# frankyangdev/net.jgp.labs.sparkdq4ml

Hardware: AMD Instinct MI355X
Metric: rows/sec LinearRegression.fit, 1e8x32 synthetic, at 1/2/4/8 MI355X (higher is better)
Workload: dtype bf16; 1 GPU; model=LinearRegression(normal equations) d=32, global_batch=100000000, seq_len=32, parallelism=dp1, rows_per_gpu=100000000, device=cuda:0, storage=bf16, fit_mode=async

## Files before the change

net/jgp/labs/sparkdq4ml_amd/ops/csrc/hip/gram.h:

```cpp
#pragma once
#ifndef __HIPCC_RTC__
#include <hip/hip_runtime.h>

#include <cstdint>
#endif

namespace dq4ml {

enum GramMode : int { GRAM_F64 = 0, GRAM_F32 = 1, GRAM_BF16 = 2, GRAM_FP8 = 3, GRAM_F32S = 4 };

struct GramArgs {
  const void* X;
  int64_t ld;
  int d;
  int64_t n;
  int xdt;
  const void* y;
  int ydt;
  const void* w;
  int wdt;
  const uint8_t* sel;
  double* partials;
  int P;
  int64_t spw;
  int64_t nsuper;
  int tiled;
  const void* colp[8];
  int coldt[8];
  int cols;
  const int64_t* srcs;
  int interleave;
  const int64_t* rawtab;
  const float* xshift;
};

#ifndef __HIPCC_RTC__
int64_t tiled_elems(int d, int64_t n);

int gram_interleave();
void tile_bf16(const void* X, int xdt, int64_t ld, int d, int64_t n, void* out, hipStream_t st,
               const float* shift = nullptr);

int64_t gram_partial_stride(int mode, int d);
int gram_default_blocks(int64_t n);
int gram_plan_blocks(int mode, int d, int64_t n, int xdt, int xmode);
void gram_tall(int mode, GramArgs a, int xmode, int blocks, double* out, hipStream_t st, bool reduce = true);
void gram_reduce(int mode, const double* partials, int blocks, int d, double* out, hipStream_t st);
void stats_unshift(double* flat, const float* shift, int d, hipStream_t st);

void gram_window_fold(const double* part, int64_t rows, int gw, double* flat, hipStream_t st);

bool gram_stream_ok(int mode, const GramArgs& a);
int gram_stream_blocks(int mode, int d, int64_t n, int xdt);
void gram_stream(int mode, GramArgs a, int xmode, int blocks, double* out, hipStream_t st, bool reduce = true);

struct PackSrcG {
// ... 12 lines not shown
```

net/jgp/labs/sparkdq4ml_amd/ops/csrc/hip/gram.hip:

```cpp
#include <hip/hip_runtime.h>

#include <cstdlib>

#include "common.h"
#include "gram.h"

namespace dq4ml {

namespace {

constexpr int kBlock = 256;
constexpr int kWavesPerBlock = kBlock / kWave;
template <int NT, int XMODE, bool HALF = false>
struct BF16Geom {
  static constexpr int kBlock = (NT == 1 && XMODE == 0 && !HALF) ? 1024 : 512;
  static constexpr int kWaves = kBlock / kWave;
  static constexpr int kMinBlocks = HALF ? 2 : 1;
};
static int bf16_block(int, int) { return 512; }

__device__ __forceinline__ double load_as_f64(const void* p, int dt, int64_t i) {
  switch (dt) {
    case DT_F64: return reinterpret_cast<const double*>(p)[i];
    case DT_F32: return (double)reinterpret_cast<const float*>(p)[i];
// ... 14 lines not shown
  RowVals v{false, 0.0, 0.0, 0.0};
  if (r < a.n) {
    bool live = a.sel ? (a.sel[r] != 0) : true;
    if (live) {
      double w = a.w ? load_as_f64(a.w, a.wdt, r) : 1.0;
      double y = load_as_f64(a.y, a.ydt, r);
      v.live = true;
      v.w = w;
      v.y = y;
      v.wy = w * y;
    }
  }
  return v;
}

struct RowAcc {
  double cnt = 0, ws = 0, wws = 0, bs = 0, bbs = 0;
  __device__ __forceinline__ void add(const RowVals& v) {
    if (v.live) {
      cnt += 1.0;
      ws += v.w;
      wws += v.w * v.w;
      bs += v.wy;
      bbs += v.wy * v.y;
    }
  }
};

template <typename T>
__device__ __forceinline__ void load_rows32_bf16(const T* p, int64_t rows_left, bf16x8 (&fr)[4]);
// ... 80 lines not shown
  const int e = o - head, pr = e / (T * T), w = e - pr * T * T, r = w / T, cc = w - (w / T) * T;
  int I = 0, rem = pr;
  while (rem >= NT - I) {
    rem -= NT - I;
    ++I;
  }
  const int J = I + rem;
  const int64_t i = (int64_t)I * T + r, j = (int64_t)J * T + cc;
  if (i <= j && j < d) out[head + i + j * (j + 1) / 2] = t;
}

__device__ __forceinline__ void slab_put(double* p, double v) {
  __hip_atomic_store(p, v, __ATOMIC_RELAXED, __HIP_MEMORY_SCOPE_AGENT);
}

template <typename TX, int NT, int XMODE, bool TILED, bool HALF = false>
__global__ __launch_bounds__((BF16Geom<NT, XMODE, HALF>::kBlock), (BF16Geom<NT, XMODE, HALF>::kMinBlocks)) void
gram_tall_bf16_kernel(GramArgs a) {
  typedef BF16Geom<NT, XMODE, HALF> Geo;
  constexpr int NPAIR = NT * (NT + 1) / 2;
  extern __shared__ __attribute__((aligned(16))) unsigned char smem[];
  const int lane = threadIdx.x & 63;
  const int wave = threadIdx.x >> 6;
  const int f = lane & 31, h = lane >> 5;
  __bf16* wl = reinterpret_cast<__bf16*>(smem) + wave * (4 * 64);
  float* wrow = reinterpret_cast<float*>(smem + Geo::kWaves * 4 * 64 * 2) + wave * 64;

  f32x16 acc[NPAIR];
  f32x16 accw[NT];
#pragma unroll
  for (int p = 0; p < NPAIR; ++p) acc[p] = f32x16{};
#pragma unroll
  for (int t = 0; t < NT; ++t) accw[t] = f32x16{};
  RowAcc ra;

  const TX* X = reinterpret_cast<const TX*>(a.X);
  const TX* fp[NT];
  bool fvalid[NT];
#pragma unroll
  for (int t = 0; t < NT; ++t) {
    const int feat = t * 32 + f;
    fvalid[t] = feat < a.d;
    fp[t] = X + (int64_t)(fvalid[t] ? feat : 0) * a.ld + 32 * h;
  }

  const int64_t gw = (int64_t)blockIdx.x * Geo::kWaves + wave;
  const int64_t total_waves = (int64_t)gridDim.x * Geo::kWaves;
  int64_t s0 = gw * a.spw;
  int64_t s1 = s0 + a.spw;
  if (s1 > a.nsuper) s1 = a.nsuper;
  const bool do_tail = (gw == total_waves - 1) && (a.n > a.nsuper * 64);

  auto compute = [&](int64_t r0, bf16x8 (&fr)[NT][4]) {
    RowVals rv = row_vals(a, r0 + lane);
    ra.add(rv);
    {
      const float w_hi = (float)(__bf16)(float)rv.w;
      const __bf16 wy_hi = (__bf16)(float)rv.wy;
      wl[0 * 64 + lane] = (__bf16)(float)rv.w;
      wl[1 * 64 + lane] = (__bf16)(float)(rv.w - (double)w_hi);
      wl[2 * 64 + lane] = wy_hi;
      wl[3 * 64 + lane] = (__bf16)(float)(rv.wy - (double)(float)wy_hi);
      if (XMODE == 2) wrow[lane] = (float)rv.w;
    }
    const uint64_t live_bits = __ballot(rv.live);
    __builtin_amdgcn_wave_barrier();
    bf16x8 wf[4];
#pragma unroll
    for (int i = 0; i < 4; ++i) wf[i] = bf16x8{};
// ... 15 lines not shown
      for (int t = 0; t < NT; ++t) weight_frags(frw[t], wrow + 32 * h);
    }
    int p = 0;
#pragma unroll
    for (int I = 0; I < NT; ++I)
#pragma unroll
      for (int J = I; J < NT; ++J, ++p)
#pragma unroll
        for (int i = 0; i < 4; ++i) acc[p] = __builtin_amdgcn_mfma_f32_32x32x16_bf16(fr[I][i], frw[J][i], acc[p], 0, 0, 0);
#pragma unroll
    for (int t = 0; t < NT; ++t)
#pragma unroll
      for (int i = 0; i < 4; ++i) accw[t] = __builtin_amdgcn_mfma_f32_32x32x16_bf16(fr[t][i], wf[i], accw[t], 0, 0, 0);
    __builtin_amdgcn_wave_barrier();
  };
  auto load = [&](int64_t r0, int64_t rows_left, bf16x8 (&fr)[NT][4]) {
    if constexpr (TILED) {
      const u32x4* q = reinterpret_cast<const u32x4*>(a.X) + ((r0 >> 6) * NT) * 4 * 64 + lane;
#pragma unroll
      for (int t = 0; t < NT; ++t)
#pragma unroll
        for (int i = 0; i < 4; ++i) fr[t][i] = __builtin_bit_cast(bf16x8, __builtin_nontemporal_load(q + (t * 4 + i) * 64));
      return;
    }
#pragma unroll
    for (int t = 0; t < NT; ++t) {
      if (fvalid[t]) {
        load_rows32_bf16<TX>(fp[t] + r0, rows_left, fr[t]);
      } else {
#pragma unroll
        for (int i = 0; i < 4; ++i) fr[t][i] = bf16x8{};
      }
    }
  };

  if (a.interleave) {
    if (gw < a.nsuper) {
      bf16x8 cur[NT][4], nxt[NT][4];
      load(gw * 64, 64, cur);
      for (int64_t s = gw; s < a.nsuper; s += total_waves) {
        if (s + total_waves < a.nsuper) load((s + total_waves) * 64, 64, nxt);
        compute(s * 64, cur);
#pragma unroll
        for (int t = 0; t < NT; ++t)
#pragma unroll
          for (int i = 0; i < 4; ++i) cur[t][i] = nxt[t][i];
      }
    }
  } else if (s0 < s1) {
    bf16x8 cur[NT][4], nxt[NT][4];
    load(s0 * 64, 64, cur);
    for (int64_t s = s0; s < s1; ++s) {
      if (s + 1 < s1) load((s + 1) * 64, 64, nxt);
      compute(s * 64, cur);
#pragma unroll
      for (int t = 0; t < NT; ++t)
#pragma unroll
        for (int i = 0; i < 4; ++i) cur[t][i] = nxt[t][i];
    }
  }
  if (do_tail) {
    bf16x8 tl[NT][4];
    const int64_t r0 = a.nsuper * 64;
    load(r0, a.n - (r0 + 32 * h), tl);
    compute(r0, tl);
  }

  constexpr int W = Geo::kWaves;
  constexpr int NV = (NPAIR + NT) * 16;
  const int d = a.d;
  double sc[5] = {ra.cnt, ra.ws, ra.wws, ra.bs, ra.bbs};
#pragma unroll
  for (int k = 0; k < 5; ++k) sc[k] = wave_sum_f64(sc[k]);
  __syncthreads();
  float* tr = reinterpret_cast<float*>(smem);
  double* scl = reinterpret_cast<double*>(smem + (size_t)(W / 2) * NV * 64 * sizeof(float));
// ... 711 lines not shown
        for (int j = 0; j < 8; ++j) e[j] = (r + j < n) ? X[(int64_t)f * ld + r + j] : (uint16_t)0;
        v = __builtin_bit_cast(u32x4, e);
      }
      if (shift) {
        const float sh = shift[f];
        bf16x8 b = __builtin_bit_cast(bf16x8, v);
#pragma unroll
        for (int j = 0; j < 8; ++j) b[j] = (r + j < n) ? (__bf16)((float)b[j] - sh) : (__bf16)0.0f;
        v = __builtin_bit_cast(u32x4, b);
      }
    }
    reinterpret_cast<u32x4*>(out)[c] = v;
  }
}

__global__ __launch_bounds__(256) void unshift_aa_kernel(double* __restrict__ flat, const float* __restrict__ shift,
                                                        int d) {
  const double W = flat[1];
  const double* as = flat + 5;
  double* aa = flat + 5 + 2 * (int64_t)d;
  const int64_t tot = (int64_t)d * (d + 1) / 2;
  for (int64_t e = (int64_t)blockIdx.x * blockDim.x + threadIdx.x; e < tot; e += (int64_t)gridDim.x * blockDim.x) {
    int64_t j = (int64_t)((sqrt(8.0 * (double)e + 1.0) - 1.0) * 0.5);
    while (j * (j + 1) / 2 > e) --j;
    while ((j + 1) * (j + 2) / 2 <= e) ++j;
    const int64_t i = e - j * (j + 1) / 2;
    const double si = (double)shift[i], sj = (double)shift[j];
    aa[e] += si * as[j] + sj * as[i] + si * sj * W;
  }
}
// ... 31 lines not shown
  const int64_t nchunks = nsup * NT * 256;
  int64_t g = (nchunks + 255) / 256;
  if (g > 8192) g = 8192;
  if (g < 1) g = 1;
  uint16_t* o = reinterpret_cast<uint16_t*>(out);
  switch (xdt) {
    case DT_BF16: hipLaunchKernelGGL(tile_bf16_kernel<uint16_t>, dim3(g), dim3(256), 0, st, (const uint16_t*)X, ld, d, n, NT, nsup, o, shift); break;
    case DT_F32: hipLaunchKernelGGL(tile_bf16_kernel<float>, dim3(g), dim3(256), 0, st, (const float*)X, ld, d, n, NT, nsup, o, shift); break;
    case DT_F64: hipLaunchKernelGGL(tile_bf16_kernel<double>, dim3(g), dim3(256), 0, st, (const double*)X, ld, d, n, NT, nsup, o, shift); break;
    case DT_I32: hipLaunchKernelGGL(tile_bf16_kernel<int32_t>, dim3(g), dim3(256), 0, st, (const int32_t*)X, ld, d, n, NT, nsup, o, shift); break;
    default: throw std::invalid_argument("tile_bf16: unsupported dtype");
  }
  DQ_HIP_CHECK(hipGetLastError());
}

int64_t gram_partial_stride(int mode, int d) {
  if (mode == GRAM_F64) {
    const int NT = (d + 15) / 16;
    return 5 + 2 * (int64_t)d + (int64_t)NT * (NT + 1) / 2 * 256;
  }
  const int NT = (d + 31) / 32;
  return 5 + 2 * (int64_t)d + (int64_t)NT * (NT + 1) / 2 * 1024;
}

int gram_default_blocks(int64_t n) {
  const int64_t nsuper = (n + 63) / 64;
  int64_t blocks = (nsuper + 8 * kWavesPerBlock - 1) / (8 * kWavesPerBlock);
  if (blocks > 1024) blocks = 1024;
  if (blocks < 1) blocks = 1;
  return (int)blocks;
// ... 12 lines not shown
static size_t bf16_lds(int d, int xmode) {
  const int W = bf16_block(d, xmode) / kWave;
  const int NT = (d + 31) / 32;
  const size_t stripes = (size_t)W * (4 * 64 * 2 + 64 * 4);
  const size_t tree = (size_t)(W / 2) * ((NT * (NT + 1) / 2 + NT) * 16) * 64 * sizeof(float) + (size_t)W * 5 * 8;
  return tree > stripes ? tree : stripes;
}

static size_t f64_lds(int d) {
  size_t lds = kWavesPerBlock * (128 + 16 * kStageLd) * sizeof(double);
  const size_t red = (size_t)gram_partial_stride(GRAM_F64, d) * sizeof(double);
  return red > lds ? red : lds;
}

template <typename F>
static void with_kernel(int mode, int xdt, int d, int xmode, bool tiled, F&& f) {
  if (mode == GRAM_BF16) {
    const int NT = (d + 31) / 32;
#define DQ_BF16_CASE(TX, NTV, TL)                                                 \
    if (xmode == 0 && NTV == 1) return f(gram_tall_bf16_kernel<TX, 1, 0, TL, true>); \
    if (xmode == 0) return f(gram_tall_bf16_kernel<TX, NTV, 0, TL>);              \
    if (xmode == 1) return f(gram_tall_bf16_kernel<TX, NTV, 1, TL>);              \
    return f(gram_tall_bf16_kernel<TX, NTV, 2, TL>);
    if (xdt == DT_BF16 && tiled) { if (NT == 1) { DQ_BF16_CASE(uint16_t, 1, true) } else { DQ_BF16_CASE(uint16_t, 2, true) } }
    if (tiled) throw std::invalid_argument("gram_tall: tiled storage must be bf16");
    if (xdt == DT_BF16) { if (NT == 1) { DQ_BF16_CASE(uint16_t, 1, false) } else { DQ_BF16_CASE(uint16_t, 2, false) } }
    if (xdt == DT_F32) { if (NT == 1) { DQ_BF16_CASE(float, 1, false) } else { DQ_BF16_CASE(float, 2, false) } }
    if (xdt == DT_F64) { if (NT == 1) { DQ_BF16_CASE(double, 1, false) } else { DQ_BF16_CASE(double, 2, false) } }
#undef DQ_BF16_CASE
    throw std::invalid_argument("gram_tall(bf16): unsupported feature dtype");
  }
  if (mode == GRAM_F64) {
    const int NT = (d + 15) / 16;
#define DQ_F64_CASE(TX)                                        \
    switch (NT) {                                              \
      case 1: return f(gram_tall_f64_kernel<TX, 1>);           \
      case 2: return f(gram_tall_f64_kernel<TX, 2>);           \
      case 3: return f(gram_tall_f64_kernel<TX, 3>);           \
      default: return f(gram_tall_f64_kernel<TX, 4>);          \
    }
    if (xdt == DT_F64) { DQ_F64_CASE(double) }
    if (xdt == DT_F32) { DQ_F64_CASE(float) }
#undef DQ_F64_CASE
// ... 64 lines not shown
int gram_plan_blocks(int mode, int d, int64_t n, int xdt, int xmode) {
  if (mode == GRAM_F32 || mode == GRAM_F32S || (use_stream() && ((mode == GRAM_F64 && !use_skinny(mode, d, xdt, 0) &&
                                              (xdt == DT_F64 || xdt == DT_F32)) ||
                                             (mode == GRAM_BF16 && xdt == DT_F32))))
    return gram_stream_blocks(mode, d, n, xdt);
  if (use_skinny(mode, d, xdt, 0)) {
    int full = 1;
    with_skinny(xdt, d, [&](auto kern) { full = occupancy_blocks(kern, 0, kBlock); });
    int64_t want = (n + (int64_t)kBlock * 4 * 8 - 1) / ((int64_t)kBlock * 4 * 8);
    if (want < 1) want = 1;
    return (int)(want < full ? want : full);
  }
  const size_t lds = mode == GRAM_BF16 ? bf16_lds(d, xmode) : f64_lds(d);
  int full = 1;
  const int block = mode == GRAM_BF16 ? bf16_block(d, xmode) : kBlock;
  with_kernel(mode, xdt, d, xmode, false, [&](auto kern) { full = occupancy_blocks(kern, lds, block); });
  const int64_t nsuper = (n + 63) / 64;
  const int wpb = block / kWave;
  int64_t want = (nsuper + 4 * wpb - 1) / (4 * wpb);
  if (want < 1) want = 1;
  return (int)(want < full ? want : full);
}

void gram_window_fold(const double* part, int64_t rows, int gw, double* flat, hipStream_t st) {
  if (gw < 1 || rows < 0) throw std::invalid_argument("gram_window_fold: bad shape");
  hipLaunchKernelGGL(window_fold_kernel, dim3(gw), dim3(256), 0, st, part, rows, gw, flat);
  DQ_HIP_CHECK(hipGetLastError());
}

void gram_reduce(int mode, const double* partials, int blocks, int d, double* out, hipStream_t st) {
  const int T = mode == GRAM_F64 ? 16 : 32;
// ... 7 lines not shown
  return 1;
}

void gram_tall(int mode, GramArgs a, int xmode, int blocks, double* out, hipStream_t st, bool reduce) {
  if (a.d < 1 || a.d > 64) throw std::invalid_argument("gram_tall: d must be in [1, 64]");
  if (blocks < 1) throw std::invalid_argument("gram_tall: blocks must be >= 1");
  a.nsuper = a.n / 64;
  const int block = mode == GRAM_BF16 ? bf16_block(a.d, xmode) : kBlock;
  const int64_t total_waves = (int64_t)blocks * (block / kWave);
  a.spw = (a.nsuper + total_waves - 1) / total_waves;
  if (a.spw < 1) a.spw = 1;
  a.interleave = gram_interleave();
  a.P = (int)gram_partial_stride(mode, a.d);
  const size_t lds = mode == GRAM_BF16 ? bf16_lds(a.d, xmode) : f64_lds(a.d);
  if (a.tiled && mode != GRAM_BF16) throw std::invalid_argument("gram_tall: tiled storage needs bf16 mode");
  if (a.xshift) {
    if (!((mode == GRAM_F32 || mode == GRAM_BF16 || mode == GRAM_F32S) && a.xdt == DT_F32 && !a.tiled && a.cols == 0 &&
          gram_stream_ok(mode, a)))
      throw std::invalid_argument("gram_tall: a feature shift needs 16-byte aligned f32 features (stream kernel)");
    gram_stream(mode, a, 1, blocks, out, st, reduce);
    return;
  }
  if (a.cols > 0) {
    if (mode != GRAM_F64 || a.cols != a.d || a.d > kSkinnyMaxD || a.tiled)
      throw std::invalid_argument("gram_tall: columnar sources need f64 mode and d <= 8");
    with_skinny_cols(a, [&](auto kern) { hipLaunchKernelGGL(kern, dim3(blocks), dim3(kBlock), 0, st, a); });
  } else if (use_skinny(mode, a.d, a.xdt, a.tiled)) {
    with_skinny(a.xdt, a.d, [&](auto kern) { hipLaunchKernelGGL(kern, dim3(blocks), dim3(kBlock), 0, st, a); });
  } else if ((mode == GRAM_F32 || mode == GRAM_F32S ||
              (use_stream() && (mode == GRAM_F64 || (mode == GRAM_BF16 && a.xdt == DT_F32)))) &&
             gram_stream_ok(mode, a)) {
    gram_stream(mode, a, xmode, blocks, out, st, reduce);
    return;
  } else if (mode == GRAM_F32 || mode == GRAM_F32S) {
    throw std::invalid_argument("gram_tall(f32): needs 16-byte aligned f32 features and f32/f64 labels");
  } else {
    with_kernel(mode, a.xdt, a.d, xmode, a.tiled != 0,
                [&](auto kern) { hipLaunchKernelGGL(kern, dim3(blocks), dim3(block), lds, st, a); });
  }
  DQ_HIP_CHECK(hipGetLastError());
  if (reduce) gram_reduce(mode, a.partials, blocks, a.d, out, st);
}

static size_t cols_lds(int NT) {
  const size_t bufs = 2 * ((size_t)NT * 4 * 64 * 16 + 4 * 64 * 2);
  const size_t tree = (size_t)2 * ((NT * (NT + 1) / 2 + NT) * 16) * 64 * sizeof(float) + 4 * 5 * sizeof(double);
  return bufs > tree ? bufs : tree;
}

template <typename F>
static void with_cols_kernel(int NT, int sdt, int ydt, F&& f) {
#define DQ_COLS(NTV, YT)                                                 \
// ... 44 lines not shown
```

net/jgp/labs/sparkdq4ml_amd/ops/csrc/hip/module.cpp:

```cpp
#include <map>
#include <utility>
#include <vector>

#include <pybind11/pybind11.h>
#include <pybind11/stl.h>

#include "common.h"
#include "csv_scan.h"
#include "dqvm.h"
#include "gram.h"
#include "gram_folds.h"
#include "quantile.h"
#include "gram_wide.h"
#include "gram_syrk.h"
#include "wls_small.h"
#include "wls_large.h"
#include "rowops.h"
#include "lsq.h"

namespace py = pybind11;
using namespace dq4ml;

template <typename T>
static T* P(uintptr_t p) {
// ... 71 lines not shown
          a.tiled = tiled;
          a.xshift = P<const float>(xshift);
          a.X = P<const void>(X);
          a.ld = ld;
          a.d = d;
          a.n = n;
          a.xdt = xdt;
          a.y = P<const void>(y);
          a.ydt = ydt;
          a.w = P<const void>(w);
          a.wdt = wdt;
          a.sel = P<const uint8_t>(sel);
          a.partials = P<double>(partials);
          gram_tall(mode, a, xmode, blocks, P<double>(out), as_stream(stream), reduce);
        });
  m.def("gram_stream_cols",
        [](int mode, uintptr_t srcs, int d, int64_t n, int xdt, uintptr_t y, int ydt, uintptr_t w, int wdt,
           uintptr_t sel, uintptr_t partials, int blocks, uintptr_t out, uintptr_t stream, uintptr_t xshift) {
          GramArgs a{};
          a.srcs = P<const int64_t>(srcs);
          a.xshift = P<const float>(xshift);
          a.d = d;
          a.n = n;
          a.xdt = xdt;
          a.y = P<const void>(y);
          a.ydt = ydt;
          a.w = P<const void>(w);
          a.wdt = wdt;
          a.sel = P<const uint8_t>(sel);
          a.partials = P<double>(partials);
// ... 437 lines not shown
```

net/jgp/labs/sparkdq4ml_amd/ops/device.py:

```python
from __future__ import annotations

import functools
from dataclasses import dataclass
import os
from typing import List, Optional

import numpy as np
import torch

from ..parallel import comm
from ..runtime import faststream
from . import native

__all__ = ["dtype_code", "gram_stats", "compact_indices", "pack_columns", "predict", "regression_metrics",
           "GRAM_MODES", "quantiles"]

_DT = {torch.float64: 0, torch.float32: 1, torch.bfloat16: 2, torch.int32: 3, torch.int64: 4, torch.uint8: 5,
       torch.bool: 5, torch.float16: 6}
GRAM_MODES = {"fp64": 0, "fp32": 1, "bf16": 2, "fp8": 3, "fp32split": 4}
_plan_cache = {}


_gram_reserve = int(os.environ.get("DQ4ML_GRAM_RESERVE_CUS", "-1"))
_cus_cache = {}
# ... 66 lines not shown
            raise ValueError(f"tensors on different devices: {dev} vs {t.device}")


def _feature_view(X: torch.Tensor, align_elems: int):
    if X.dim() != 2:
        raise ValueError("feature matrix must be 2-D [d, n]")
    d, n = X.shape
    if X.stride(1) != 1 or (d > 1 and X.stride(0) % align_elems) or X.data_ptr() % 16:
        ld = (n + 63) // 64 * 64
        buf = torch.zeros(d, ld, dtype=X.dtype, device=X.device)
        buf[:, :n] = X
        return buf, ld
    return X, (X.stride(0) if d > 1 else max(n, 1))


from .layout import TiledBF16, TiledWide
from .shift import column_shift

FP8_MAX = 448.0


def _auto_shift(parts, shift, uniform=False):
    if isinstance(shift, str):
        if shift != "auto":
            raise ValueError(f"shift: 'auto', None or an ops.shift.Shift, not {shift!r}")
        return column_shift(parts, uniform=uniform)
    return shift


def _sptr(shift) -> int:
    return 0 if shift is None else shift.dev.data_ptr()


def _unshift(h, out: torch.Tensor, shift, d: int) -> torch.Tensor:
    if shift is not None:
        h.stats_unshift(out.data_ptr(), shift.dev.data_ptr(), int(d), _stream())
    return out


def tile_bf16(X: torch.Tensor, shift="auto") -> TiledBF16:
    h = native.hip()
    _check_dev(X)
    d, n = X.shape
    if X.stride(1) != 1:
        X = X.contiguous()
    shift = _auto_shift([X], shift)
    ld = X.stride(0) if d > 1 else max(n, 1)
    buf = torch.empty(int(h.tiled_elems(d, n)), dtype=torch.bfloat16, device=X.device)
    h.tile_bf16(X.data_ptr(), dtype_code(X), int(ld), int(d), int(n), buf.data_ptr(), _stream(), _sptr(shift))
    return TiledBF16(buf, d, n, shift)


class DeferredGram:

    is_cuda = True

    def __init__(self, h, mode, partials, nb, d, out, shift=None):
        self._h, self.mode, self.partials, self.nb, self.d, self.out = h, mode, partials, nb, d, out
        self.shift = shift
        self.device = out.device

    def finish(self) -> torch.Tensor:
        st = faststream.current(faststream.dev_index(self.device))
        self.partials.record_stream(st)
        self.out.record_stream(st)
# ... 27 lines not shown
        return _gram_syrk(h, X, y, w, sel, compute_f64=mode == 0)
    if mode in (1, 4):
        if X.dtype not in (torch.float32, torch.float64):
            X = X.to(torch.float32)
        if X.dtype != torch.float32 or d <= 8:
            mode = 0
    if mode == 2 and X.dtype not in (torch.bfloat16, torch.float32, torch.float64):
        X = X.to(torch.float32)
    if mode == 0 and X.dtype not in (torch.float64, torch.float32):
        X = X.to(torch.float64)
    shift = None
    if mode in (1, 2, 4):
        shift = column_shift([X])
        if shift is not None and X.dtype != torch.float32:
            if mode == 2 and w is None:
                return _gram_tiled(h, tile_bf16(X, shift), y, None, sel, False, blocks, defer)
            X = X.to(torch.float32).contiguous()
    align = 16 // X.element_size()
    Xv, ld = _feature_view(X, align)
    y = y.contiguous()
    if y.dtype not in (torch.float64, torch.float32):
        y = y.to(torch.float64)
    if w is not None:
        w = w.contiguous()
        if w.dtype not in (torch.float64, torch.float32):
            w = w.to(torch.float64)
    if sel is not None:
        sel = sel.contiguous()
        if sel.dtype != torch.bool:
            sel = sel.to(torch.bool)
    if y.numel() != n or (w is not None and w.numel() != n) or (sel is not None and sel.numel() != n):
# ... 275 lines not shown
def _prep_rows(y, w, sel, n):
    y = y.contiguous()
    if y.dtype not in (torch.float64, torch.float32):
        y = y.to(torch.float64)
    if w is not None:
        w = w.contiguous()
        if w.dtype not in (torch.float64, torch.float32):
            w = w.to(torch.float64)
    if sel is not None:
        sel = sel.contiguous().to(torch.bool)
    if y.numel() != n or (w is not None and w.numel() != n) or (sel is not None and sel.numel() != n):
        raise ValueError("gram_stats: row-count mismatch")
    return y, w, sel


class TiledGramPlan:

    __slots__ = ("h", "T", "y", "w", "sel", "d", "nb", "flat_len", "part_len", "dev", "pre", "post")

    def __init__(self, h, T: "TiledBF16", y, w, sel, x_zero_dead):
        d, n = T.d, T.n
        if d > 64:
            raise ValueError("tiled Gram supports d <= 64")
        _check_dev(T.buf, y, w, sel)
        y, w, sel = _prep_rows(y, w, sel, n)
        xmode = 2 if w is not None else (1 if (sel is not None and not x_zero_dead) else 0)
        self.h, self.T, self.y, self.w, self.sel, self.d, self.dev = h, T, y, w, sel, d, T.device
        self.nb = int(_plan_blocks(h, 2, d, n, 2, xmode))
        self.flat_len = 5 + 2 * d + d * (d + 1) // 2
        self.part_len = self.nb * int(h.gram_partial_stride(2, d))
        self.pre = (2, T.buf.data_ptr(), 0, int(d), int(n), 2, y.data_ptr(), dtype_code(y), _ptr(w),
                    dtype_code(w) if w is not None else 0, _ptr(sel), xmode)

    def launch(self, stream: int, defer: bool):
        out = torch.empty(self.flat_len, dtype=torch.float64, device=self.dev)
        partials = torch.empty(self.part_len, dtype=torch.float64, device=self.dev)
        self.h.gram_tall(*self.pre, partials.data_ptr(), self.nb, out.data_ptr(), stream, 1, not defer, 0)
        sh = self.T.shift
        if defer:
            return DeferredGram(self.h, 2, partials, self.nb, self.d, out, sh)
        if sh is not None:
            self.h.stats_unshift(out.data_ptr(), sh.dev.data_ptr(), self.d, stream)
        return out


def _gram_tiled(h, T: "TiledBF16", y, w, sel, x_zero_dead, blocks, defer=False):
    d, n = T.d, T.n
    if d > 64:
        raise ValueError("tiled Gram supports d <= 64")
    _check_dev(T.buf, y, w, sel)
    y, w, sel = _prep_rows(y, w, sel, n)
    out = torch.empty(5 + 2 * d + d * (d + 1) // 2, dtype=torch.float64, device=T.device)
    xmode = 2 if w is not None else (1 if (sel is not None and not x_zero_dead) else 0)
    nb = int(blocks or _plan_blocks(h, 2, d, n, 2, xmode))
    P = int(h.gram_partial_stride(2, d))
    partials = torch.empty(nb * P, dtype=torch.float64, device=T.device)
    h.gram_tall(2, T.buf.data_ptr(), 0, int(d), int(n), 2, y.data_ptr(), dtype_code(y), _ptr(w),
                dtype_code(w) if w is not None else 0, _ptr(sel), xmode, partials.data_ptr(), nb, out.data_ptr(),
                _stream(), 1, not defer, 0)
    if defer:
        return DeferredGram(h, 2, partials, nb, d, out, T.shift)
    return _unshift(h, out, T.shift, d)


_syrk_pairs = {}


def _syrk_pair_table(P: int, dev) -> torch.Tensor:
    key = (P, str(dev))
    t = _syrk_pairs.get(key)
    if t is None:
        pairs = sorted(((i, j) for i in range(P) for j in range(i, P)), key=lambda p: _morton(*p))
        t = _syrk_pairs[key] = _h2d(np.asarray(pairs, dtype=np.int32).reshape(-1), dev)
    return t
# ... 944 lines not shown
```

net/jgp/labs/sparkdq4ml_amd/ops/layout.py:

```python
from __future__ import annotations

import torch

__all__ = ["TiledBF16", "tiled_offsets"]


def tiled_offsets(feats: torch.Tensor, rows: torch.Tensor, d: int) -> torch.Tensor:
    NT = (d + 31) // 32
    s = rows >> 6
    h = (rows >> 5) & 1
    i = (rows >> 3) & 3
    j = rows & 7
    t = feats >> 5
    lane = 32 * h + (feats & 31)
    return ((((s * NT + t) * 4 + i) * 64 + lane) << 3) + j


def _unshift_rows(vals: torch.Tensor, shift) -> torch.Tensor:
    if shift is None:
        return vals
    return vals.to(torch.float32) + shift.dev.to(vals.device).unsqueeze(1)


class TiledBF16:
    def __init__(self, buf: torch.Tensor, d: int, n: int, shift=None):
        assert buf.dtype == torch.bfloat16 and buf.dim() == 1
        self.buf, self.d, self.n = buf, int(d), int(n)
        self.shift = shift

    @property
    def shape(self):
        return (self.d, self.n)

    @property
    def device(self):
        return self.buf.device

    @property
    def dtype(self):
        return torch.bfloat16

    @property
    def is_cuda(self):
# ... 81 lines not shown
```

Baseline: 102.3 billion rows/s.

## Add exponent-range packed companion for tiled bf16 storage to cut Gram read traffic

Adds a pack pass that, for each 64-row by 32-feature tile whose bf16 exponents span at most 16 values, stores the tile in 3/4 of the bytes (exponent offset from a per-tile base byte), plus a directory byte per tile. The tiled Gram kernel gets a PACKED variant that reads the directory, loads three dwords instead of four for packed tiles, and unpacks with bit ops before the MFMAs. It also double-buffers tile loads and reads labels as raw bits. The aim is to cut HBM read volume in a bandwidth-bound Gram pass. The cost is extra unpack ALU work, an extra directory read, and a pack pass plus a companion buffer kept alongside the original tiles, which raises total memory use.

```diff
diff --git a/net/jgp/labs/sparkdq4ml_amd/ops/csrc/hip/gram.h b/net/jgp/labs/sparkdq4ml_amd/ops/csrc/hip/gram.h
--- a/net/jgp/labs/sparkdq4ml_amd/ops/csrc/hip/gram.h
+++ b/net/jgp/labs/sparkdq4ml_amd/ops/csrc/hip/gram.h
@@ -32,6 +32,8 @@
   int interleave;
   const int64_t* rawtab;
   const float* xshift;
+  const uint32_t* xpack;
+  const uint8_t* xdir;
 };
 
 #ifndef __HIPCC_RTC__
@@ -40,6 +42,9 @@
 int gram_interleave();
 void tile_bf16(const void* X, int xdt, int64_t ld, int d, int64_t n, void* out, hipStream_t st,
                const float* shift = nullptr);
+
+void pack_tiles(const void* tiles, int d, int64_t n, uint8_t* dir, uint32_t* slots, uint32_t* npacked,
+                hipStream_t st);
 
 int64_t gram_partial_stride(int mode, int d);
 int gram_default_blocks(int64_t n);
diff --git a/net/jgp/labs/sparkdq4ml_amd/ops/csrc/hip/gram.hip b/net/jgp/labs/sparkdq4ml_amd/ops/csrc/hip/gram.hip
--- a/net/jgp/labs/sparkdq4ml_amd/ops/csrc/hip/gram.hip
+++ b/net/jgp/labs/sparkdq4ml_amd/ops/csrc/hip/gram.hip
@@ -52,6 +52,43 @@
   return v;
 }
 
+struct LabelBits {
+  uint32_t lo, hi;
+};
+
+__device__ __forceinline__ LabelBits label_bits(const GramArgs& a, int64_t r) {
+  LabelBits b{0u, 0u};
+  if (r < a.n) {
+    if (a.ydt == DT_F64) {
+      const u32x2 v = reinterpret_cast<const u32x2*>(a.y)[r];
+      b.lo = v[0];
+      b.hi = v[1];
+    } else {
+      b.lo = reinterpret_cast<const uint32_t*>(a.y)[r];
+    }
+  }
+  return b;
+}
+
+template <bool WEIGHTS>
+__device__ __forceinline__ RowVals row_vals(const GramArgs& a, int64_t r, LabelBits b) {
+  RowVals v{false, 0.0, 0.0, 0.0};
+  if (r < a.n) {
+    bool live = a.sel ? (a.sel[r] != 0) : true;
+    if (live) {
+      double w = 1.0;
+      if constexpr (WEIGHTS) w = a.w ? load_as_f64(a.w, a.wdt, r) : 1.0;
+      double y = a.ydt == DT_F64 ? __longlong_as_double(((long long)b.hi << 32) | (long long)b.lo)
+                                 : (double)__uint_as_float(b.lo);
+      v.live = true;
+      v.w = w;
+      v.y = y;
+      v.wy = w * y;
+    }
+  }
+  return v;
+}
+
 struct RowAcc {
   double cnt = 0, ws = 0, wws = 0, bs = 0, bbs = 0;
   __device__ __forceinline__ void add(const RowVals& v) {
@@ -162,9 +199,27 @@
   __hip_atomic_store(p, v, __ATOMIC_RELAXED, __HIP_MEMORY_SCOPE_AGENT);
 }
 
-template <typename TX, int NT, int XMODE, bool TILED, bool HALF = false>
+__device__ __forceinline__ void unpack_tile(const u32x4 (&raw)[4], uint32_t B2, bf16x8 (&fr)[4]) {
+#pragma unroll
+  for (int i = 0; i < 4; ++i) {
+    const uint32_t d0 = raw[0][i], d1 = raw[1][i], d2 = raw[2][i];
+    uint32_t q = (d0 >> 11) & 0x000F000Fu;
+    q |= (d1 >> 7) & 0x00F000F0u;
+    q |= (d2 >> 3) & 0x07000700u;
+    q |= (d2 & 0x40004000u) << 1;
+    u32x4 r;
+    r[0] = (d0 & 0x87FF87FFu) + B2;
+    r[1] = (d1 & 0x87FF87FFu) + B2;
+    r[2] = (d2 & 0x87FF87FFu) + B2;
+    r[3] = q + B2;
+    fr[i] = __builtin_bit_cast(bf16x8, r);
+  }
+}
+
+template <typename TX, int NT, int XMODE, bool TILED, bool HALF = false, bool PACKED = false>
 __global__ __launch_bounds__((BF16Geom<NT, XMODE, HALF>::kBlock), (BF16Geom<NT, XMODE, HALF>::kMinBlocks)) void
 gram_tall_bf16_kernel(GramArgs a) {
+  static_assert(!PACKED || TILED, "the packed companion belongs to tiled storage");
   typedef BF16Geom<NT, XMODE, HALF> Geo;
   constexpr int NPAIR = NT * (NT + 1) / 2;
   extern __shared__ __attribute__((aligned(16))) unsigned char smem[];
@@ -192,15 +247,14 @@
     fp[t] = X + (int64_t)(fvalid[t] ? feat : 0) * a.ld + 32 * h;
   }
 
-  const int64_t gw = (int64_t)blockIdx.x * Geo::kWaves + wave;
+  const int64_t gw = (int64_t)blockIdx.x * Geo::kWaves + (PACKED ? __builtin_amdgcn_readfirstlane(wave) : wave);
   const int64_t total_waves = (int64_t)gridDim.x * Geo::kWaves;
   int64_t s0 = gw * a.spw;
   int64_t s1 = s0 + a.spw;
   if (s1 > a.nsuper) s1 = a.nsuper;
   const bool do_tail = (gw == total_waves - 1) && (a.n > a.nsuper * 64);
 
-  auto compute = [&](int64_t r0, bf16x8 (&fr)[NT][4]) {
-    RowVals rv = row_vals(a, r0 + lane);
+  auto compute_rv = [&](const RowVals& rv, bf16x8 (&fr)[NT][4]) {
     ra.add(rv);
     {
       const float w_hi = (float)(__bf16)(float)rv.w;
@@ -246,6 +300,7 @@
       for (int i = 0; i < 4; ++i) accw[t] = __builtin_amdgcn_mfma_f32_32x32x16_bf16(fr[t][i], wf[i], accw[t], 0, 0, 0);
     __builtin_amdgcn_wave_barrier();
   };
+  auto compute = [&](int64_t r0, bf16x8 (&fr)[NT][4]) { compute_rv(row_vals(a, r0 + lane), fr); };
   auto load = [&](int64_t r0, int64_t rows_left, bf16x8 (&fr)[NT][4]) {
     if constexpr (TILED) {
       const u32x4* q = reinterpret_cast<const u32x4*>(a.X) + ((r0 >> 6) * NT) * 4 * 64 + lane;
@@ -266,6 +321,89 @@
     }
   };
 
+  auto pk_dir = [&](int64_t s, uint32_t (&dv)[NT]) {
+    const uint32_t* words = reinterpret_cast<const uint32_t*>(a.xdir);
+#pragma unroll
+    for (int t = 0; t < NT; ++t) dv[t] = words[(s * NT + t) >> 2];
+  };
+  auto dir_bytes = [&](int64_t s, const uint32_t (&dv)[NT], int (&db)[NT]) {
+#pragma unroll
+    for (int t = 0; t < NT; ++t)
+      db[t] = (int)((__builtin_amdgcn_readfirstlane(dv[t]) >> (8 * (int)((s * NT + t) & 3))) & 0xFFu);
+  };
+  auto pk_y = [&](int64_t s) { return label_bits(a, s * 64 + lane); };
+  auto pk_load = [&](int64_t s, const int (&db)[NT], u32x4 (&raw)[NT][4], int ln) {
+#pragma unroll
+    for (int t = 0; t < NT; ++t) {
+      const bool pk = db[t] != 0xFF;
+      const int64_t e = s * NT + t;
+      const u32x4* q = (pk ? reinterpret_cast<const u32x4*>(a.xpack) + e * 3 * 64
+                           : reinterpret_cast<const u32x4*>(a.X) + e * 4 * 64) + ln;
+#pragma unroll
+      for (int k = 0; k < 3; ++k) raw[t][k] = __builtin_nontemporal_load(q + k * 64);
+      if (!pk) raw[t][3] = __builtin_nontemporal_load(q + 3 * 64);
+    }
+  };
+  auto pk_compute = [&](int64_t s, const int (&db)[NT], const u32x4 (&raw)[NT][4], LabelBits yb) {
+    bf16x8 fr[NT][4];
+#pragma unroll
+    for (int t = 0; t < NT; ++t) {
+      if (db[t] != 0xFF) {
+        unpack_tile(raw[t], (uint32_t)db[t] * 0x00800080u, fr[t]);
+      } else {
+#pragma unroll
+        for (int i = 0; i < 4; ++i) fr[t][i] = __builtin_bit_cast(bf16x8, raw[t][i]);
+      }
+    }
+    compute_rv(row_vals<XMODE == 2>(a, s * 64 + lane, yb), fr);
+  };
+
+  if constexpr (PACKED) {
+    const int64_t step = a.interleave ? total_waves : 1;
+    const int64_t end = a.interleave ? a.nsuper : s1;
+    int64_t s = a.interleave ? gw : s0;
+    auto pk_next = [&](int64_t s, const uint32_t (&dv)[NT], int (&db)[NT], u32x4 (&raw)[NT][4], LabelBits& yb) {
+      const bool more = s + step < end;
+      dir_bytes(s + step, dv, db);
+#pragma unroll
+      for (int t = 0; t < NT; ++t) db[t] = more ? db[t] : 0;
+      pk_load(more ? s + step : 0, db, raw, more ? lane : 0);
+      yb = pk_y(more ? s + step : s);
+      return more;
+    };
+    if (s < end) {
+      u32x4 A[NT][4], B[NT][4];
+      int dA[NT], dB[NT];
+      uint32_t dv[NT];
+      LabelBits yA, yB;
+      pk_dir(s, dv);
+      dir_bytes(s, dv, dA);
+      pk_load(s, dA, A, lane);
+      yA = pk_y(s);
+      if (s + step < end) pk_dir(s + step, dv);
+      for (;;) {
+        bool more = pk_next(s, dv, dB, B, yB);
+        if (s + 2 * step < end) pk_dir(s + 2 * step, dv);
+        pk_compute(s, dA, A, yA);
+        if (!more) break;
+        s += step;
+        more = pk_next(s, dv, dA, A, yA);
+        if (s + 2 * step < end) pk_dir(s + 2 * step, dv);
+        pk_compute(s, dB, B, yB);
+        if (!more) break;
+        s += step;
+      }
+    }
+    if (do_tail) {
+      u32x4 A[NT][4];
+      int dA[NT];
+      uint32_t dv[NT];
+      pk_dir(a.nsuper, dv);
+      dir_bytes(a.nsuper, dv, dA);
+      pk_load(a.nsuper, dA, A, lane);
+      pk_compute(a.nsuper, dA, A, pk_y(a.nsuper));
+    }
+  } else
   if (a.interleave) {
     if (gw < a.nsuper) {
       bf16x8 cur[NT][4], nxt[NT][4];
@@ -291,7 +429,7 @@
         for (int i = 0; i < 4; ++i) cur[t][i] = nxt[t][i];
     }
   }
-  if (do_tail) {
+  if (!PACKED && do_tail) {
     bf16x8 tl[NT][4];
     const int64_t r0 = a.nsuper * 64;
     load(r0, a.n - (r0 + 32 * h), tl);
@@ -1033,6 +1171,53 @@
   }
 }
 
+__global__ __launch_bounds__(256) void pack_tiles_kernel(const u32x4* __restrict__ tiles, int64_t nent,
+                                                        uint8_t* __restrict__ dir, u32x4* __restrict__ slots,
+                                                        uint32_t* __restrict__ npacked) {
+  const int lane = threadIdx.x & 63;
+  const int64_t w0 = (int64_t)blockIdx.x * (blockDim.x >> 6) + (threadIdx.x >> 6);
+  const int64_t nw = (int64_t)gridDim.x * (blockDim.x >> 6);
+  uint32_t mine = 0;
+  for (int64_t e = w0; e < nent; e += nw) {
+    u32x4 r[4];
+    uint32_t emin = 255u, emax = 0u;
+#pragma unroll
+    for (int i = 0; i < 4; ++i) {
+      r[i] = tiles[(e * 4 + i) * 64 + lane];
+#pragma unroll
+      for (int j = 0; j < 4; ++j) {
+        const uint32_t lo = (r[i][j] >> 7) & 0xFFu, hi = (r[i][j] >> 23) & 0xFFu;
+        emin = min(emin, min(lo, hi));
+        emax = max(emax, max(lo, hi));
+      }
+    }
+#pragma unroll
+    for (int o = 32; o >= 1; o >>= 1) {
+      emin = min(emin, (uint32_t)__shfl_xor((int)emin, o, 64));
+      emax = max(emax, (uint32_t)__shfl_xor((int)emax, o, 64));
+    }
+    const bool ok = emax - emin <= 15u && emin <= 254u;
+    if (lane == 0) dir[e] = ok ? (uint8_t)emin : (uint8_t)0xFF;
+    u32x4 D[3] = {u32x4{0u, 0u, 0u, 0u}, u32x4{0u, 0u, 0u, 0u}, u32x4{0u, 0u, 0u, 0u}};
+    if (ok) {
+      ++mine;
+      const uint32_t B2 = emin * 0x00800080u;
+#pragma unroll
+      for (int i = 0; i < 4; ++i) {
+        const uint32_t p3 = (r[i][3] & 0x7FFF7FFFu) - B2;
+#pragma unroll
+        for (int k = 0; k < 3; ++k) D[k][i] = (r[i][k] & 0x80008000u) | ((r[i][k] & 0x7FFF7FFFu) - B2);
+        D[0][i] |= (p3 & 0x000F000Fu) << 11;
+        D[1][i] |= (p3 & 0x00F000F0u) << 7;
+        D[2][i] |= ((p3 & 0x07000700u) << 3) | ((r[i][3] & 0x80008000u) >> 1);
+      }
+    }
+#pragma unroll
+    for (int k = 0; k < 3; ++k) slots[(e * 3 + k) * 64 + lane] = D[k];
+  }
+  if (lane == 0 && mine) atomicAdd(npacked, mine);
+}
+
 __global__ __launch_bounds__(256) void unshift_aa_kernel(double* __restrict__ flat, const float* __restrict__ shift,
                                                         int d) {
   const double W = flat[1];
@@ -1094,6 +1279,18 @@
   DQ_HIP_CHECK(hipGetLastError());
 }
 
+void pack_tiles(const void* tiles, int d, int64_t n, uint8_t* dir, uint32_t* slots, uint32_t* npacked,
+                hipStream_t st) {
+  if (d < 1 || d > 64) throw std::invalid_argument("pack_tiles: d must be in [1, 64]");
+  const int64_t nent = ((n + 63) / 64) * ((d + 31) / 32);
+  if (nent < 1) return;
+  int64_t g = (nent + 3) / 4;
+  if (g > 16384) g = 16384;
+  hipLaunchKernelGGL(pack_tiles_kernel, dim3(g), dim3(256), 0, st, reinterpret_cast<const u32x4*>(tiles), nent, dir,
+                     reinterpret_cast<u32x4*>(slots), npacked);
+  DQ_HIP_CHECK(hipGetLastError());
+}
+
 int64_t gram_partial_stride(int mode, int d) {
   if (mode == GRAM_F64) {
     const int NT = (d + 15) / 16;
@@ -1136,19 +1333,21 @@
 }
 
 template <typename F>
-static void with_kernel(int mode, int xdt, int d, int xmode, bool tiled, F&& f) {
+static void with_kernel(int mode, int xdt, int d, int xmode, bool tiled, bool packed, F&& f) {
   if (mode == GRAM_BF16) {
     const int NT = (d + 31) / 32;
-#define DQ_BF16_CASE(TX, NTV, TL)                                                 \
-    if (xmode == 0 && NTV == 1) return f(gram_tall_bf16_kernel<TX, 1, 0, TL, true>); \
-    if (xmode == 0) return f(gram_tall_bf16_kernel<TX, NTV, 0, TL>);              \
-    if (xmode == 1) return f(gram_tall_bf16_kernel<TX, NTV, 1, TL>);              \
-    return f(gram_tall_bf16_kernel<TX, NTV, 2, TL>);
-    if (xdt == DT_BF16 && tiled) { if (NT == 1) { DQ_BF16_CASE(uint16_t, 1, true) } else { DQ_BF16_CASE(uint16_t, 2, true) } }
+#define DQ_BF16_CASE(TX, NTV, TL, PK)                                                    \
+    if (xmode == 0 && NTV == 1) return f(gram_tall_bf16_kernel<TX, 1, 0, TL, true, PK>); \
+    if (xmode == 0) return f(gram_tall_bf16_kernel<TX, NTV, 0, TL, false, PK>);          \
+    if (xmode == 1) return f(gram_tall_bf16_kernel<TX, NTV, 1, TL, false, PK>);          \
+    return f(gram_tall_bf16_kernel<TX, NTV, 2, TL, false, PK>);
+    if (packed && !(xdt == DT_BF16 && tiled)) throw std::invalid_argument("gram_tall: packed tiles need tiled bf16 storage");
+    if (packed) { if (NT == 1) { DQ_BF16_CASE(uint16_t, 1, true, true) } else { DQ_BF16_CASE(uint16_t, 2, true, true) } }
+    if (xdt == DT_BF16 && tiled) { if (NT == 1) { DQ_BF16_CASE(uint16_t, 1, true, false) } else { DQ_BF16_CASE(uint16_t, 2, true, false) } }
     if (tiled) throw std::invalid_argument("gram_tall: tiled storage must be bf16");
-    if (xdt == DT_BF16) { if (NT == 1) { DQ_BF16_CASE(uint16_t, 1, false) } else { DQ_BF16_CASE(uint16_t, 2, false) } }
-    if (xdt == DT_F32) { if (NT == 1) { DQ_BF16_CASE(float, 1, false) } else { DQ_BF16_CASE(float, 2, false) } }
-    if (xdt == DT_F64) { if (NT == 1) { DQ_BF16_CASE(double, 1, false) } else { DQ_BF16_CASE(double, 2, false) } }
+    if (xdt == DT_BF16) { if (NT == 1) { DQ_BF16_CASE(uint16_t, 1, false, false) } else { DQ_BF16_CASE(uint16_t, 2, false, false) } }
+    if (xdt == DT_F32) { if (NT == 1) { DQ_BF16_CASE(float, 1, false, false) } else { DQ_BF16_CASE(float, 2, false, false) } }
+    if (xdt == DT_F64) { if (NT == 1) { DQ_BF16_CASE(double, 1, false, false) } else { DQ_BF16_CASE(double, 2, false, false) } }
 #undef DQ_BF16_CASE
     throw std::invalid_argument("gram_tall(bf16): unsupported feature dtype");
   }
@@ -1243,7 +1442,7 @@
   const size_t lds = mode == GRAM_BF16 ? bf16_lds(d, xmode) : f64_lds(d);
   int full = 1;
   const int block = mode == GRAM_BF16 ? bf16_block(d, xmode) : kBlock;
-  with_kernel(mode, xdt, d, xmode, false, [&](auto kern) { full = occupancy_blocks(kern, lds, block); });
+  with_kernel(mode, xdt, d, xmode, false, false, [&](auto kern) { full = occupancy_blocks(kern, lds, block); });
   const int64_t nsuper = (n + 63) / 64;
   const int wpb = block / kWave;
   int64_t want = (nsuper + 4 * wpb - 1) / (4 * wpb);
@@ -1281,6 +1480,12 @@
   a.P = (int)gram_partial_stride(mode, a.d);
   const size_t lds = mode == GRAM_BF16 ? bf16_lds(a.d, xmode) : f64_lds(a.d);
   if (a.tiled && mode != GRAM_BF16) throw std::invalid_argument("gram_tall: tiled storage needs bf16 mode");
+  if ((a.xpack != nullptr) != (a.xdir != nullptr) || (a.xpack && !(a.tiled && mode == GRAM_BF16)))
+    throw std::invalid_argument("gram_tall: packed tiles come as a slot buffer plus a directory, with tiled bf16 storage");
+  if (a.xpack && a.w && xmode != 2) throw std::invalid_argument("gram_tall: packed tiles with weights need xmode 2");
+  if (a.xpack && ((a.ydt != DT_F32 && a.ydt != DT_F64) || (reinterpret_cast<uintptr_t>(a.xdir) & 3) ||
+                  (reinterpret_cast<uintptr_t>(a.xpack) & 15)))
+    throw std::invalid_argument("gram_tall: packed tiles need f32 / f64 labels, a word-aligned directory and 16-byte aligned slots");
   if (a.xshift) {
     if (!((mode == GRAM_F32 || mode == GRAM_BF16 || mode == GRAM_F32S) && a.xdt == DT_F32 && !a.tiled && a.cols == 0 &&
           gram_stream_ok(mode, a)))
@@ -1302,7 +1507,7 @@
   } else if (mode == GRAM_F32 || mode == GRAM_F32S) {
     throw std::invalid_argument("gram_tall(f32): needs 16-byte aligned f32 features and f32/f64 labels");
   } else {
-    with_kernel(mode, a.xdt, a.d, xmode, a.tiled != 0,
+    with_kernel(mode, a.xdt, a.d, xmode, a.tiled != 0, a.xpack != nullptr,
                 [&](auto kern) { hipLaunchKernelGGL(kern, dim3(blocks), dim3(block), lds, st, a); });
   }
   DQ_HIP_CHECK(hipGetLastError());
diff --git a/net/jgp/labs/sparkdq4ml_amd/ops/csrc/hip/module.cpp b/net/jgp/labs/sparkdq4ml_amd/ops/csrc/hip/module.cpp
--- a/net/jgp/labs/sparkdq4ml_amd/ops/csrc/hip/module.cpp
+++ b/net/jgp/labs/sparkdq4ml_amd/ops/csrc/hip/module.cpp
@@ -109,6 +109,29 @@
           a.partials = P<double>(partials);
           gram_tall(mode, a, xmode, blocks, P<double>(out), as_stream(stream), reduce);
         });
+  m.def("gram_tall_packed",
+        [](uintptr_t X, uintptr_t xpack, uintptr_t xdir, int d, int64_t n, uintptr_t y, int ydt, uintptr_t w, int wdt,
+           uintptr_t sel, int xmode, uintptr_t partials, int blocks, uintptr_t out, uintptr_t stream, bool reduce) {
+          GramArgs a{};
+          a.tiled = 1;
+          a.X = P<const void>(X);
+          a.xpack = P<const uint32_t>(xpack);
+          a.xdir = P<const uint8_t>(xdir);
+          a.d = d;
+          a.n = n;
+          a.xdt = DT_BF16;
+          a.y = P<const void>(y);
+          a.ydt = ydt;
+          a.w = P<const void>(w);
+          a.wdt = wdt;
+          a.sel = P<const uint8_t>(sel);
+          a.partials = P<double>(partials);
+          gram_tall(GRAM_BF16, a, xmode, blocks, P<double>(out), as_stream(stream), reduce);
+        });
+  m.def("pack_tiles", [](uintptr_t tiles, int d, int64_t n, uintptr_t dir, uintptr_t slots, uintptr_t npacked,
+                         uintptr_t stream) {
+    pack_tiles(P<const void>(tiles), d, n, P<uint8_t>(dir), P<uint32_t>(slots), P<uint32_t>(npacked), as_stream(stream));
+  });
   m.def("gram_stream_cols",
         [](int mode, uintptr_t srcs, int d, int64_t n, int xdt, uintptr_t y, int ydt, uintptr_t w, int wdt,
            uintptr_t sel, uintptr_t partials, int blocks, uintptr_t out, uintptr_t stream, uintptr_t xshift) {
diff --git a/net/jgp/labs/sparkdq4ml_amd/ops/device.py b/net/jgp/labs/sparkdq4ml_amd/ops/device.py
--- a/net/jgp/labs/sparkdq4ml_amd/ops/device.py
+++ b/net/jgp/labs/sparkdq4ml_amd/ops/device.py
@@ -104,7 +104,7 @@
     return X, (X.stride(0) if d > 1 else max(n, 1))
 
 
-from .layout import TiledBF16, TiledWide
+from .layout import SLOT_DWORDS, PackedTiles, TiledBF16, TiledWide
 from .shift import column_shift
 
 FP8_MAX = 448.0
@@ -128,7 +128,36 @@
     return out
 
 
-def tile_bf16(X: torch.Tensor, shift="auto") -> TiledBF16:
+PACK_MIN_ROWS = 3_000_000
+
+
+def pack_tiles(T: TiledBF16) -> PackedTiles:
+    h = native.hip()
+    _check_dev(T.buf)
+    if T.d > 64:
+        raise ValueError("packed tiles support d <= 64")
+    ne = int(h.tiled_elems(T.d, T.n)) // 2048
+    dirb = torch.empty((ne + 3) // 4 * 4, dtype=torch.uint8, device=T.device)[:ne]
+    slots = torch.empty(ne * SLOT_DWORDS, dtype=torch.int32, device=T.device)
+    cnt = torch.zeros(1, dtype=torch.int32, device=T.device)
+    if ne:
+        h.pack_tiles(T.buf.data_ptr(), int(T.d), int(T.n), dirb.data_ptr(), slots.data_ptr(), cnt.data_ptr(), _stream())
+    return PackedTiles(dirb, slots, int(cnt.item()))
+
+
+def _maybe_pack(T: TiledBF16, pack) -> TiledBF16:
+    if pack is True:
+        T.packed = pack_tiles(T)
+    elif pack == "auto":
+        if os.environ.get("DQ4ML_TILE_PACK", "1") != "0" and T.n >= PACK_MIN_ROWS and T.d <= 64:
+            p = pack_tiles(T)
+            T.packed = p if 2 * p.npacked >= p.dir.numel() else None
+    elif pack is not False:
+        raise ValueError(f"pack: True, False or 'auto', not {pack!r}")
+    return T
+
+
+def tile_bf16(X: torch.Tensor, shift="auto", pack="auto") -> TiledBF16:
     h = native.hip()
     _check_dev(X)
     d, n = X.shape
@@ -138,7 +167,7 @@
     ld = X.stride(0) if d > 1 else max(n, 1)
     buf = torch.empty(int(h.tiled_elems(d, n)), dtype=torch.bfloat16, device=X.device)
     h.tile_bf16(X.data_ptr(), dtype_code(X), int(ld), int(d), int(n), buf.data_ptr(), _stream(), _sptr(shift))
-    return TiledBF16(buf, d, n, shift)
+    return _maybe_pack(TiledBF16(buf, d, n, shift), pack)
 
 
 class DeferredGram:
@@ -196,7 +225,7 @@
         shift = column_shift([X])
         if shift is not None and X.dtype != torch.float32:
             if mode == 2 and w is None:
-                return _gram_tiled(h, tile_bf16(X, shift), y, None, sel, False, blocks, defer)
+                return _gram_tiled(h, tile_bf16(X, shift, pack=False), y, None, sel, False, blocks, defer)
             X = X.to(torch.float32).contiguous()
     align = 16 // X.element_size()
     Xv, ld = _feature_view(X, align)
@@ -502,9 +531,16 @@
     return y, w, sel
 
 
+def _tiled_pre(T: "TiledBF16", y, w, sel, xmode):
+    rows = (y.data_ptr(), dtype_code(y), _ptr(w), dtype_code(w) if w is not None else 0, _ptr(sel), xmode)
+    if T.packed is not None:
+        return (T.buf.data_ptr(), T.packed.a.data_ptr(), T.packed.dir.data_ptr(), int(T.d), int(T.n)) + rows
+    return (2, T.buf.data_ptr(), 0, int(T.d), int(T.n), 2) + rows
+
+
 class TiledGramPlan:
 
-    __slots__ = ("h", "T", "y", "w", "sel", "d", "nb", "flat_len", "part_len", "dev", "pre", "post")
+    __slots__ = ("h", "T", "y", "w", "sel", "d", "nb", "flat_len", "part_len", "dev", "pre", "post", "packed")
 
     def __init__(self, h, T: "TiledBF16", y, w, sel, x_zero_dead):
         d, n = T.d, T.n
@@ -517,13 +553,16 @@
         self.nb = int(_plan_blocks(h, 2, d, n, 2, xmode))
         self.flat_len = 5 + 2 * d + d * (d + 1) // 2
         self.part_len = self.nb * int(h.gram_partial_stride(2, d))
-        self.pre = (2, T.buf.data_ptr(), 0, int(d), int(n), 2, y.data_ptr(), dtype_code(y), _ptr(w),
-                    dtype_code(w) if w is not None else 0, _ptr(sel), xmode)
+        self.pre = _tiled_pre(T, y, w, sel, xmode)
+        self.packed = T.packed is not None
 
     def launch(self, stream: int, defer: bool):
         out = torch.empty(self.flat_len, dtype=torch.float64, device=self.dev)
         partials = torch.empty(self.part_len, dtype=torch.float64, device=self.dev)
-        self.h.gram_tall(*self.pre, partials.data_ptr(), self.nb, out.data_ptr(), stream, 1, not defer, 0)
+        if self.packed:
+            self.h.gram_tall_packed(*self.pre, partials.data_ptr(), self.nb, out.data_ptr(), stream, not defer)
+        else:
+            self.h.gram_tall(*self.pre, partials.data_ptr(), self.nb, out.data_ptr(), stream, 1, not defer, 0)
         sh = self.T.shift
         if defer:
             return DeferredGram(self.h, 2, partials, self.nb, self.d, out, sh)
@@ -543,9 +582,11 @@
     nb = int(blocks or _plan_blocks(h, 2, d, n, 2, xmode))
     P = int(h.gram_partial_stride(2, d))
     partials = torch.empty(nb * P, dtype=torch.float64, device=T.device)
-    h.gram_tall(2, T.buf.data_ptr(), 0, int(d), int(n), 2, y.data_ptr(), dtype_code(y), _ptr(w),
-                dtype_code(w) if w is not None else 0, _ptr(sel), xmode, partials.data_ptr(), nb, out.data_ptr(),
-                _stream(), 1, not defer, 0)
+    pre = _tiled_pre(T, y, w, sel, xmode)
+    if T.packed is not None:
+        h.gram_tall_packed(*pre, partials.data_ptr(), nb, out.data_ptr(), _stream(), not defer)
+    else:
+        h.gram_tall(*pre, partials.data_ptr(), nb, out.data_ptr(), _stream(), 1, not defer, 0)
     if defer:
         return DeferredGram(h, 2, partials, nb, d, out, T.shift)
     return _unshift(h, out, T.shift, d)
diff --git a/net/jgp/labs/sparkdq4ml_amd/ops/layout.py b/net/jgp/labs/sparkdq4ml_amd/ops/layout.py
--- a/net/jgp/labs/sparkdq4ml_amd/ops/layout.py
+++ b/net/jgp/labs/sparkdq4ml_amd/ops/layout.py
@@ -2,7 +2,7 @@
 
 import torch
 
-__all__ = ["TiledBF16", "tiled_offsets"]
+__all__ = ["TiledBF16", "tiled_offsets", "PackedTiles", "pack_reference", "unpack_reference"]
 
 
 def tiled_offsets(feats: torch.Tensor, rows: torch.Tensor, d: int) -> torch.Tensor:
@@ -22,11 +22,67 @@
     return vals.to(torch.float32) + shift.dev.to(vals.device).unsqueeze(1)
 
 
+RAW_ENTRY = 0xFF
+SLOT_DWORDS = 768
+
+
+class PackedTiles:
+
+    def __init__(self, dir: torch.Tensor, a: torch.Tensor, npacked: int):
+        assert dir.dtype == torch.uint8 and a.dtype == torch.int32 and a.numel() == dir.numel() * SLOT_DWORDS
+        self.dir, self.a, self.npacked = dir, a, int(npacked)
+
+    @property
+    def fraction(self) -> float:
+        return self.npacked / max(1, self.dir.numel())
+
+
+def _halfwords(buf: torch.Tensor) -> torch.Tensor:
+    return (buf.view(torch.int16).to(torch.int32) & 0xFFFF).view(-1, 4, 64, 8)
+
+
+def _to_i16(hw: torch.Tensor) -> torch.Tensor:
+    return (((hw + 0x8000) & 0xFFFF) - 0x8000).to(torch.int16)
+
+
+def pack_reference(buf: torch.Tensor) -> PackedTiles:
+    v = _halfwords(buf)
+    e = (v >> 7) & 0xFF
+    emin, emax = e.amin(dim=(1, 2, 3)), e.amax(dim=(1, 2, 3))
+    ok = ((emax - emin) <= 15) & (emin <= 254)
+    base = torch.where(ok, emin, torch.zeros_like(emin)).view(-1, 1, 1, 1)
+    p = (v & 0x7FFF) - (base << 7)
+    sg = v & 0x8000
+    p3, s3 = p[..., 6:8], sg[..., 6:8]
+    nib = torch.stack([p3 & 0xF, (p3 >> 4) & 0xF, ((p3 >> 8) & 0x7) | (s3 >> 12)], dim=-2)
+    hw = (sg[..., :6] | p[..., :6]).reshape(-1, 4, 64, 3, 2) | (nib << 11)
+    hw = hw.permute(0, 3, 2, 1, 4)
+    hw = torch.where(ok.view(-1, 1, 1, 1, 1), hw, torch.zeros_like(hw))
+    a = _to_i16(hw).contiguous().view(-1).view(torch.int32)
+    d8 = torch.where(ok, emin, torch.full_like(emin, RAW_ENTRY)).to(torch.uint8)
+    return PackedTiles(d8, a, int(ok.sum()))
+
+
+def unpack_reference(packed: PackedTiles, buf: torch.Tensor) -> torch.Tensor:
+    ne = packed.dir.numel()
+    hw = (packed.a.view(torch.int16).to(torch.int32) & 0xFFFF).view(ne, 3, 64, 4, 2).permute(0, 3, 2, 1, 4)
+    base = packed.dir.to(torch.int32).view(-1, 1, 1, 1, 1) << 7
+    main = (hw & 0x87FF) + base
+    nib = (hw >> 11) & 0xF
+    p3 = nib[..., 0, :] | (nib[..., 1, :] << 4) | ((nib[..., 2, :] & 0x7) << 8)
+    r3 = (p3 | ((nib[..., 2, :] & 0x8) << 12)) + base[..., 0, :]
+    dec = torch.cat([main.reshape(ne, 4, 64, 6), r3], dim=-1)
+    raw = _halfwords(buf)
+    out = torch.where((packed.dir != RAW_ENTRY).view(-1, 1, 1, 1), dec, raw)
+    return _to_i16(out).view(-1).view(torch.bfloat16)
+
+
 class TiledBF16:
-    def __init__(self, buf: torch.Tensor, d: int, n: int, shift=None):
+    def __init__(self, buf: torch.Tensor, d: int, n: int, shift=None, packed: "PackedTiles" = None):
         assert buf.dtype == torch.bfloat16 and buf.dim() == 1
         self.buf, self.d, self.n = buf, int(d), int(n)
         self.shift = shift
+        self.packed = packed
 
     @property
     def shape(self):
```

Measured after the change: 121.2 billion rows/s, median of 6. 1.18x the previous value.
